# GogoRit/llm-inference-lab

Measured on AMD Instinct MI355X. Metric: accepted tokens/sec + acceptance-rate, Llama-3.2-3B/1B K=4 @1/2/4/8 GPU, higher is better.
Workload: dtype bf16; 1 GPU; llama-3.2-3b target + llama-3.2-1b draft, K=4, batch 1/GPU, greedy, prompt 32 ids, hipGraph step, weights: synthetic; K=4, batch_per_gpu=1, global_batch=1, prompt_len=32, parallelism=dp1

## Files before the change

llm-inference-lab_amd/csrc/debug_env.h:

```cpp
#pragma once

namespace sd {
namespace debug_env {

constexpr const char* kNoPersist = "SPECDEC_NO_PERSIST";
constexpr const char* kPersistMaxT = "SPECDEC_PERSIST_MAX_T";
constexpr const char* kPersistTaps = "SPECDEC_PERSIST_TAPS";
constexpr const char* kPersistDropWg = "SPECDEC_PERSIST_TEST_DROP_WG";
constexpr const char* kNoFwd0Select = "SPECDEC_NO_FWD0_SELECT";
constexpr const char* kMaxPassTokens = "SPECDEC_MAX_PASS_TOKENS";
constexpr const char* kNoDirect = "SPECDEC_NO_DIRECT";
constexpr const char* kNoPipe = "SPECDEC_NO_PIPE";
constexpr const char* kNoAttnSplit = "SPECDEC_NO_ATTN_SPLIT";
constexpr const char* kNoGemmPrefill = "SPECDEC_NO_GEMM_PREFILL";
constexpr const char* kPrefillMinTokens = "SPECDEC_PREFILL_MIN_TOKENS";
constexpr const char* kMedusaPerHead = "SPECDEC_MEDUSA_PER_HEAD";
constexpr const char* kGemvTimeline = "SPECDEC_GEMV_TIMELINE";
constexpr const char* kProbeHot = "SPECDEC_PROBE_HOT";
constexpr const char* kProbeNoXstat = "SPECDEC_PROBE_NO_XSTAT";

}
}
```

llm-inference-lab_amd/csrc/engine.hip:

```cpp

#include <hip/hip_runtime.h>

#include <stdlib.h>

#include <new>
#include <vector>

#include "engine.h"
#include "persist.h"
#include "prefill_gemm.h"

struct sd_model {
  sd_model_config cfg;
  std::vector<sd_layer_weights> layers;
  uint16_t* k_cache = nullptr;
  uint16_t* v_cache = nullptr;
  int B = 0, Lmax = 0;
  const int32_t* block_table = nullptr;
  int page_shift = 0, max_pages = 0, n_pages = 0;
  uint16_t* x = nullptr;
  uint16_t* q = nullptr;
  uint16_t* attn = nullptr;
  uint16_t* act = nullptr;
  int32_t* probe_pos = nullptr;
  float* attn_ws = nullptr;
  unsigned* attn_cnt = nullptr;
  float* xstat = nullptr;
  float* part_val = nullptr;
  int small_t = sd::kGemvMaxT;
  int max_t = sd::kGemvMaxT;
  int* part_idx = nullptr;
  int head_grid = 0;
  const int32_t* skip_k = nullptr;
  int skip_i = 0;
  std::vector<const void*> packed;
  std::vector<const float*> scales;
  const void* mat(int index, const void* row_major) const { return packed.empty() ? row_major : packed[index]; }
  int is_packed() const { return packed.empty() ? 0 : 1; }
  int w8() const { return scales.empty() ? 0 : 1; }
  const float* scale(int index) const { return scales.empty() ? nullptr : scales[index]; }
  int persist_t = 0;
  bool persist_taps = true;
  sd::PersistOp* p_ops = nullptr;
  unsigned long long* p_gran = nullptr;
  unsigned p_gran_parity = 0;
  unsigned* p_sync = nullptr;
  unsigned long long* p_debug = nullptr;
  void* prefill_ws = nullptr;
  int prefill_backend = SD_PREFILL_AUTO;
  int64_t prefill_count[4] = {0, 0, 0, 0};
  sd::NativePlan native_plan;
  void* score_ws = nullptr;
  unsigned* host_status = nullptr;
  int persist_cap = 0;
  int len_hint = 0;
  int ctx_limit = 0;
  ~sd_model() {
// ... 53 lines not shown
  const int d = c.d_model, HqD = c.n_heads * c.head_dim, ff = c.d_ff;
  const struct { const uint16_t* x; int x_stride; uint16_t* out; int out_stride; } rows[5] = {
      {m->x, d, m->q, HqD}, {m->attn, HqD, m->x, d}, {m->x, d, m->act, ff}, {m->act, ff, m->x, d}, {m->x, d, nullptr, 0}};
  a.x = rows[which].x;
  a.x_stride = rows[which].x_stride;
  a.out = rows[which].out;
  a.out_stride = rows[which].out_stride;
  a.out_dtype = SD_BF16;
  if (which == 4) {
    a.part_val = m->part_val;
    a.part_idx = m->part_idx;
  }
  return a;
}

static int forward_pass(sd_model* m, const int32_t* tokens, int tok_stride, const int32_t* pos_base,
                        int pos_off, int row0, int b0, int Bc, int Mc, int32_t* ids_out, int ids_stride,
                        void* logits_out, int logits_dtype, int logits_stride, int skip_head,
                        hipStream_t st) {
  const sd_model_config& c = m->cfg;
  const int T = Bc * Mc;
  const int d = c.d_model, Hq = c.n_heads, Hkv = c.n_kv_heads, D = c.head_dim, ff = c.d_ff;
  const bool llama = (c.arch == SD_ARCH_LLAMA);

  if (persist_pass_ok(m, T, Bc, Mc)) {
    PersistArgs pa{};
    pa.ops = m->p_ops;
    pa.n_ops = 4 * c.n_layers + (skip_head ? 0 : 1);
    pa.d_model = d; pa.n_q_heads = Hq; pa.n_kv_heads = Hkv; pa.head_dim = D; pa.d_ff = ff; pa.vocab = c.vocab;
    pa.n_layers = c.n_layers; pa.max_pos = c.max_pos;
    pa.norm_eps = c.norm_eps;
    pa.attn_scale = 1.0f / sqrtf(static_cast<float>(D));
    pa.tok_emb = c.tok_emb;
    pa.rope_cos = c.rope_cos;
    pa.rope_sin = c.rope_sin;
    pa.tokens = tokens + static_cast<size_t>(b0) * tok_stride;
    pa.tok_stride = tok_stride;
    pa.pos_base = pos_base + b0;
    pa.pos_off = pos_off;
    pa.B = Bc;
    pa.M = Mc;
    const size_t row_off = static_cast<size_t>(row0 + b0) * Hkv * m->Lmax * D;
    pa.k_cache = m->k_cache + row_off;
    pa.v_cache = m->v_cache + row_off;
    pa.layer_kv = static_cast<size_t>(m->B) * Hkv * m->Lmax * D;
    pa.l_max = m->Lmax;
    pa.logits = logits_out;
    pa.logits_dtype = logits_dtype;
    pa.logits_stride = logits_stride;
    pa.part_val = m->part_val;
    pa.part_idx = m->part_idx;
    pa.x = m->x; pa.q = m->q; pa.attn = m->attn; pa.act = m->act;
    pa.gran = m->p_gran;
    pa.gran_parity = m->p_gran_parity;
    pa.sync = m->p_sync;
    pa.host_status = m->host_status;
    pa.skip_k = m->skip_k;
    pa.skip_i = m->skip_i;
    pa.taps = (m->persist_taps || skip_head) ? 1 : 0;
    pa.debug_ts = m->p_debug;
    if (int rc = launch_persist_forward(pa, st)) return rc;
    if (skip_head) return 0;
    m->head_grid = kPersistCUs;
    if (ids_out) {
      if (int rc = launch_argmax_finalize(m->part_val, m->part_idx, T, m->head_grid, Mc, ids_stride,
                                          ids_out + static_cast<size_t>(b0) * ids_stride, st, m->skip_k, m->skip_i))
        return rc;
    }
    return 0;
  }

  EmbedArgs e{};
  e.tok_emb = c.tok_emb;
  e.pos_emb = llama ? nullptr : c.pos_emb;
  e.tokens = tokens + static_cast<size_t>(b0) * tok_stride;
  e.tok_stride = tok_stride;
  e.pos_base = pos_base + b0;
  e.pos_off = pos_off;
  e.M = Mc;
  e.T = T;
  e.d = d;
  e.vocab = c.vocab;
  e.max_pos = c.max_pos;
  e.x = m->x;
  e.skip_k = m->skip_k;
  e.skip_i = m->skip_i;
  if (int rc = launch_embed(e, st)) return rc;

  const bool paged = m->block_table != nullptr;
  const size_t layer_kv = paged ? (static_cast<size_t>(m->n_pages) * Hkv * D << m->page_shift) : static_cast<size_t>(m->B) * Hkv * m->Lmax * D;
  const size_t row_kv = paged ? 0 : static_cast<size_t>(row0 + b0) * Hkv * m->Lmax * D;
  const int32_t* bt = paged ? m->block_table + static_cast<size_t>(row0 + b0) * m->max_pages : nullptr;
  const float* stat_in = nullptr;
  int stat_n = 0;
  auto publish = [&](GemvArgs& prod) {
    stat_in = nullptr;
    if (m->xstat && gemm_resid_publishes_stats(prod)) {
      prod.xstat_out = m->xstat;
      stat_in = m->xstat;
      int ppw = 1;
      stat_n = gemv_grid(prod, &ppw);
    }
  };
  for (int l = 0; l < c.n_layers; ++l) {
    uint16_t* kc = m->k_cache + l * layer_kv + row_kv;
    uint16_t* vc = m->v_cache + l * layer_kv + row_kv;
    auto layer_args = [&](int which) {
      GemvArgs g = matrix_args(m, 4 * l + which);
      g.T = T;
// ... 837 lines not shown
    if (int rc = launch_argmax_finalize(m->part_val, m->part_idx, B * K, grid, K, K + 1, s->st.verify_tok + 1, st_t)) return rc;
    if (int rc = launch_medusa_commit(s->st, st_t)) return rc;
  } else if (!s->draft && s->heads.empty()) {
    if (int rc = model_forward(s->target, s->st.verify_tok, K + 1, s->st.cur_len, 0, 0, B, 1, s->st.draft_ids, 2, nullptr, SD_BF16, 0, st_t))
      return rc;
    if (int rc = launch_medusa_fill(s->st, st_t)) return rc;
  }
  if (two) {
    SD_HIP_CHECK(hipEventRecord(s->ev_fork, st_t));
    SD_HIP_CHECK(hipStreamWaitEvent(st_d, s->ev_fork, 0));
  }
  struct TapsGuard {
    sd_model* m; bool saved;
    TapsGuard(sd_model* m_, bool v) : m(m_), saved(m_ ? m_->persist_taps : false) { if (m) m->persist_taps = v; }
    ~TapsGuard() { if (m) m->persist_taps = saved; }
  } taps_guard(s->draft, s->draft_taps);
  const bool fwd0_select = s->draft && s->st.fwd0_w && B == 1 && persist_pass_ok(s->draft, 2, 1, 2);
  const bool one_pass_d = s->draft && B * 2 <= s->draft->max_t;
  const auto finalize = [&](int M, int i, int32_t* ids, const int32_t* skip_k, int skip_i) -> int {
    if (one_pass_d)
      return launch_draft_finalize(s->draft->part_val, s->draft->part_idx, s->draft->head_grid, M, i, ids, s->st, skip_k, skip_i, st_d);
    return 0;
  };
  const bool spec = s->spec != 0;
  const int V = s->target->cfg.vocab;
  uint16_t* const q_pass = spec ? static_cast<uint16_t*>(s->spec_p) : nullptr;
  int32_t* const ids_d = (one_pass_d || spec) ? nullptr : s->st.draft_ids;
  for (int i = 0; s->draft && i < K; ++i) {
    const int M = (i == 0) ? 2 : 1;
    const int32_t* toks = (i == 0) ? s->st.tok2 : s->st.next_tok;
    const int off = (i == 0) ? -1 : i;
    s->draft->skip_k = (s->st.adaptive && i >= 1) ? s->st.k_active : nullptr;
    s->draft->skip_i = i;
    int rc_f;
    if (i == 0 && fwd0_select) {
      s->draft->skip_k = s->st.fwd0_w;
      s->draft->skip_i = 1;
      rc_f = model_forward(s->draft, toks, 2, s->st.cur_len, -1, 0, B, 2, ids_d, 2, q_pass, SD_BF16, 0, st_d);
      if (!rc_f && !spec) rc_f = finalize(2, 0, s->st.draft_ids, s->st.fwd0_w, 1);
      if (!rc_f) {
        s->draft->skip_k = s->st.fwd0_w + 1;
        rc_f = model_forward(s->draft, toks + 1, 2, s->st.cur_len, 0, 0, B, 1, ids_d ? ids_d + 1 : nullptr, 2, spec ? q_pass + V : nullptr,
                             SD_BF16, 0, st_d);
      }
      if (!rc_f && !spec) rc_f = finalize(1, 0, s->st.draft_ids + 1, s->st.fwd0_w + 1, 1);
    } else {
      rc_f = model_forward(s->draft, toks, M, s->st.cur_len, off, 0, B, M, ids_d, 2, q_pass, SD_BF16, 0, st_d);
      if (!rc_f && !spec) rc_f = finalize(M, i, s->st.draft_ids, s->draft->skip_k, i);
    }
    s->draft->skip_k = nullptr;
    if (rc_f) return rc_f;
    if (spec && s->spec_top_k > 0) {
      if (int rc = launch_spec_draft_draw_shaped(s->st, q_pass, M, M - 1, s->spec_q, i, V, s->temperature, s->spec_top_k, s->spec_top_p,
                                                 s->seed, s->draw, s->stream_id, st_d))
        return rc;
    } else if (spec) {
      if (int rc = launch_spec_draft_draw(s->st, q_pass, M, M - 1, s->spec_q, i, V, s->temperature, s->seed, s->draw, s->stream_id, st_d)) return rc;
    } else if (!one_pass_d) {
      if (int rc = launch_draft_next(M, i, s->st, st_d)) return rc;
    }
  }
  if (two) {
    SD_HIP_CHECK(hipEventRecord(s->ev_join, st_d));
    SD_HIP_CHECK(hipStreamWaitEvent(st_t, s->ev_join, 0));
  }
  const unsigned* const st_word_d = (s->draft && s->draft->p_sync) ? s->draft->p_sync + 1 : nullptr;
  const unsigned* const st_word_t = s->target->p_sync ? s->target->p_sync + 1 : nullptr;
  const bool tail = !s->sample && !spec && verify_tail_fits(s->st) && B * (K + 1) <= s->target->max_t;
  if (int rc = model_forward(s->target, s->st.verify_tok, K + 1, s->st.cur_len, 0, 0, B, K + 1, tail ? nullptr : s->st.target_ids,
                             K + 1, s->sample ? s->logits : (spec ? s->spec_p : nullptr), SD_BF16, 0, st_t))
    return rc;
  if (tail) {
    if (int rc = launch_verify_tail(s->st, s->target->part_val, s->target->part_idx, s->target->head_grid, s->mode, s->host_record, s->rec,
                                    s->step_counter, st_word_d, st_word_t, st_t))
      return rc;
    if (!s->heads.empty())
      if (int rc = enqueue_medusa_heads(s, st_t)) return rc;
    return 0;
  }
  if (s->sample) {
    if (int rc = launch_accept_len(s->st, st_t)) return rc;
    if (int rc = launch_sample_step(s->st, s->logits, s->target->cfg.vocab, s->temperature, s->top_k, s->top_p, s->seed,
                                    s->draw, s->stream_id, st_t))
      return rc;
  }
  if (spec && s->spec_top_k > 0) {
    if (int rc = launch_spec_step_shaped(s->st, s->spec_p, s->spec_q, V, s->temperature, s->spec_top_k, s->spec_top_p, s->seed, s->draw,
                                         s->stream_id, s->spec_flags, s->spec_flags + static_cast<size_t>(B) * (K + 1), st_t))
      return rc;
  } else if (spec) {
    if (int rc = launch_spec_step(s->st, s->spec_p, s->spec_q, V, s->temperature, s->seed, s->draw, s->stream_id, s->spec_flags,
                                  s->spec_flags + static_cast<size_t>(B) * (K + 1), st_t))
      return rc;
  }
// ... 394 lines not shown
}

extern "C" long sd_specdec_launches(const sd_specdec* s) { return s ? s->launches : 0; }

extern "C" int sd_specdec_wait(sd_specdec* s, long launch_index) {
  clear_error();
  SD_REQUIRE(s, "specdec_wait: NULL");
  SD_REQUIRE(launch_index >= 0 && launch_index < s->launches && launch_index + 2 >= s->launches,
             "specdec_wait: step %ld is not one of the last two launches (%ld launched)", launch_index, s->launches);
  SD_HIP_CHECK(hipEventSynchronize(s->ev_done[launch_index & 1]));
  return 0;
}

extern "C" int sd_specdec_sync(sd_specdec* s, void* stream) {
  clear_error();
  (void)s;
  SD_HIP_CHECK(hipStreamSynchronize(static_cast<hipStream_t>(stream)));
  return 0;
}

extern "C" const int32_t* sd_specdec_record(const sd_specdec* s) { return s ? s->host_record : nullptr; }

extern "C" int sd_specdec_record_ints(const sd_specdec* s) { return s ? s->rec : 0; }
```

llm-inference-lab_amd/csrc/kernels.h:

```cpp
#pragma once

#include <vector>

#include "common.h"
#include "debug_env.h"

namespace sd {

enum GemvPrologue { PRO_NONE = 0, PRO_RMSNORM = 1, PRO_LAYERNORM = 2 };
enum GemvEpilogue { EPI_QKV_ROPE = 0, EPI_RESID = 1, EPI_SWIGLU = 2, EPI_GELU = 3, EPI_ARGMAX = 4 };

constexpr int kGemvMaxT = 9;
constexpr int kSkinnyMaxT = 128;
static_assert(kSkinnyMaxT <= 255, "GemvArgs::T / M are 8-bit fields");

struct GemvArgs {
  const void* W;
  const void* x;
  void* out;
  const void* norm_w;
  const void* norm_b;
  const void* bias;
  const int32_t* x_row;
  const int32_t* skip_k;
// ... 90 lines not shown

struct AttnArgs {
  const void* q;
  const void* k_cache;
  const void* v_cache;
  void* out;
  const int32_t* pos_base;
  const int32_t* skip_k;
  int pos_off;
  int l_max;
  float scale;
  unsigned M : 8, n_q_heads : 8, n_kv_heads : 8, n_split : 8;
  unsigned head_dim : 8, page_shift : 8, skip_i : 4;
  int B;
  float* split_ws;
  unsigned* split_cnt;
  int split_slots;
  const int32_t* block_table;
};
int launch_attention(const AttnArgs& a, hipStream_t st);
constexpr int kAttnSplitSlots = 1024;
size_t attention_split_ws_bytes(int head_dim);

struct EmbedArgs {
  const void* tok_emb;
  const void* pos_emb;
  const int32_t* tokens;
  int tok_stride;
  const int32_t* pos_base;
  int pos_off, M, T, d, vocab, max_pos;
  void* x;
  const int32_t* skip_k;
  int skip_i;
};
int launch_embed(const EmbedArgs& a, hipStream_t st);

int launch_argmax_finalize(const float* part_val, const int* part_idx, int T, int grid, int M,
                           int ids_stride, int32_t* ids_out, hipStream_t st, const int32_t* skip_k = nullptr, int skip_i = 0);

}
```

llm-inference-lab_amd/csrc/misc.hip:

```cpp

#include "kernels.h"
#include "engine.h"

namespace sd {

__global__ __launch_bounds__(256) void embed_kernel(const EmbedArgs a) {
  SD_SKIP_IF_INACTIVE(a.skip_k, a.skip_i);
  const int t = blockIdx.x;
  const int b = t / a.M, m = t - b * a.M;
  int tok = a.tokens[b * a.tok_stride + m];
  tok = tok < 0 ? 0 : (tok >= a.vocab ? a.vocab - 1 : tok);
  const uint4* src = reinterpret_cast<const uint4*>(static_cast<const uint16_t*>(a.tok_emb) + static_cast<size_t>(tok) * a.d);
  uint4* dst = reinterpret_cast<uint4*>(static_cast<uint16_t*>(a.x) + static_cast<size_t>(t) * a.d);
  const int nvec = a.d >> 3;
  if (!a.pos_emb) {
    for (int v = threadIdx.x; v < nvec; v += blockDim.x) dst[v] = src[v];
    return;
  }
  int pos = a.pos_base[b] + a.pos_off + m;
  pos = pos < 0 ? 0 : (pos >= a.max_pos ? a.max_pos - 1 : pos);
  const uint4* ps = reinterpret_cast<const uint4*>(static_cast<const uint16_t*>(a.pos_emb) + static_cast<size_t>(pos) * a.d);
  for (int v = threadIdx.x; v < nvec; v += blockDim.x) {
    const uint4 e = src[v], p = ps[v];
    const uint32_t ew[4] = {e.x, e.y, e.z, e.w}, pw[4] = {p.x, p.y, p.z, p.w};
    uint32_t o[4];
#pragma unroll
    for (int j = 0; j < 4; ++j) {
      const float lo = __uint_as_float(ew[j] << 16) + __uint_as_float(pw[j] << 16);
      const float hi = __uint_as_float(ew[j] & 0xffff0000u) + __uint_as_float(pw[j] & 0xffff0000u);
      o[j] = static_cast<uint32_t>(float_to_bf16_bits(lo)) | (static_cast<uint32_t>(float_to_bf16_bits(hi)) << 16);
    }
    dst[v] = make_uint4(o[0], o[1], o[2], o[3]);
  }
}

int launch_embed(const EmbedArgs& a, hipStream_t st) {
  SD_REQUIRE(a.d % 8 == 0, "embed: d=%d must be a multiple of 8", a.d);
  hipLaunchKernelGGL(embed_kernel, dim3(a.T), dim3(256), 0, st, a);
  SD_LAUNCH_CHECK();
  return 0;
}

__device__ __forceinline__ int fold_partials(const float* pv, const int* pi, int grid, int lane) {
  float v = -INFINITY;
  int i = 0x7fffffff;
  for (int s = lane; s < grid; s += kWave) {
    const float sv = pv[s];
    const int si = pi[s];
    if (argmax_better(sv, si, v, i)) { v = sv; i = si; }
  }
  wave_reduce_argmax(v, i);
  return i;
}

__global__ __launch_bounds__(kWave) void argmax_finalize_kernel(const float* part_val, const int* part_idx,
                                                                int grid, int M, int ids_stride,
                                                                int32_t* ids, const int32_t* skip_k, int skip_i) {
  SD_SKIP_IF_INACTIVE(skip_k, skip_i);
  const int t = blockIdx.x, lane = threadIdx.x;
  const int i = fold_partials(part_val + static_cast<size_t>(t) * grid, part_idx + static_cast<size_t>(t) * grid, grid, lane);
  if (lane == 0) {
    if (M > 0) {
      const int b = t / M, m = t - b * M;
      ids[b * ids_stride + m] = i;
    } else {
      const int j = t / -M, b = t + j * M;
      ids[b * ids_stride + j] = i;
    }
  }
}

int launch_argmax_finalize(const float* part_val, const int* part_idx, int T, int grid, int M,
                           int ids_stride, int32_t* ids_out, hipStream_t st, const int32_t* skip_k, int skip_i) {
  hipLaunchKernelGGL(argmax_finalize_kernel, dim3(T), dim3(kWave), 0, st, part_val, part_idx, grid, M,
                     ids_stride, ids_out, skip_k, skip_i);
// ... 348 lines not shown
```

llm-inference-lab_amd/csrc/persist.h:

```cpp
#pragma once

#include "kernels.h"

namespace sd {

enum PersistKind { POP_QKV = 0, POP_OUT = 1, POP_GATEUP = 2, POP_DOWN = 3, POP_HEAD = 4 };

struct PersistOp {
  const void* W;
  const void* norm_w;
  unsigned pair_bytes;
  int n_pairs, ppw, tile_pairs;
  int K;
  int kind, layer;
  int pad_[5];
};
static_assert(sizeof(PersistOp) == 64, "PersistOp is read as whole 64-byte records");

constexpr int kPersistMaxT = 8;
constexpr int kPersistCUs = 256;
constexpr int kPersistMaxQkvTiles = 4;

enum PersistEdge { PE_X = 0, PE_QKV = 1, PE_ATTN = 2, PE_X2 = 3, PE_ACT = 4 };

// ... 10 lines not shown
  const int32_t* pos_base;
  int pos_off;
  int B, M;
  void* k_cache;
  void* v_cache;
  size_t layer_kv;
  int l_max;
  void* logits;
  int logits_dtype, logits_stride;
  float* part_val;
  int* part_idx;
  void* x;
  void* q;
  void* attn;
  void* act;
  unsigned long long* gran;
  unsigned gran_parity;
  unsigned off_edge[5];
  unsigned gran_unit;
  unsigned* sync;
  unsigned* host_status;
  const int32_t* skip_k;
  int skip_i;
  unsigned lds_rope, lds_resid, lds_part, lds_attn, lds_u, lds_ring;
  unsigned ring_bytes;
  unsigned u_stride;
  unsigned resid_ppw;
  int taps;
  unsigned long long* debug_ts;
};

size_t persist_workspace_bytes(const sd_model_config& c);
constexpr unsigned kGranUnitMax = 528;
bool persist_model_ok(const sd_model_config& c, bool packed, bool w8, int n_cus);
inline bool persist_cache_ok(int l_max) { return l_max >= 8 && l_max % 8 == 0; }
int persist_max_tokens(const sd_model_config& c);
int launch_persist_forward(PersistArgs a, hipStream_t st);

}
```

llm-inference-lab_amd/csrc/persist.hip:

```cpp

#include <stdlib.h>

#include "gemv_device.h"
#include "persist.h"

#ifndef SD_P_DIAG
#define SD_P_DIAG 0
#endif

namespace sd {
namespace {

constexpr unsigned kPiece = 1024;
constexpr int kChunk = 16;
constexpr int kBackoff = 2;
constexpr int kSplitSweep = 2048;
constexpr int kLeadInUnits = 96;
constexpr unsigned kUniformSites = 13;
constexpr unsigned kTimeoutTicks = 50u * 1000u * 100u;
constexpr int kPartT = kPersistMaxT;

enum : unsigned { ST_LOADER = 1u, ST_LANDED = 2u, ST_USEQ = 4u, ST_PART = 8u, ST_GRANULE = 16u, ST_ATTN = 32u };

struct PCtl {
  unsigned landed;
  unsigned consumed[3];
  unsigned abort_;
  unsigned u_seq;
  unsigned done[3];
  unsigned lead_done;
  unsigned a_seq;
  unsigned a_done[3];
  unsigned a_merged;
  unsigned g2_seq;
  unsigned a2_seq;
  unsigned nsum[2];
  unsigned nseq[2];
  unsigned gathering;
};

typedef const PersistOp __attribute__((address_space(4)))* cops_t;

__device__ __forceinline__ unsigned lds_ld(const unsigned* p) {
  const unsigned v = __hip_atomic_load(p, __ATOMIC_RELAXED, __HIP_MEMORY_SCOPE_WORKGROUP);
  asm volatile("" ::: "memory");
  return static_cast<unsigned>(__builtin_amdgcn_readfirstlane(static_cast<int>(v)));
}
__device__ __forceinline__ void lds_st(unsigned* p, unsigned v) {
  asm volatile("" ::: "memory");
  __hip_atomic_store(p, v, __ATOMIC_RELAXED, __HIP_MEMORY_SCOPE_WORKGROUP);
}

__device__ __forceinline__ void dma_piece(const char* sbase, unsigned voff, unsigned lds_dst) {
  asm volatile("s_mov_b32 m0, %2\n\ts_nop 0\n\tglobal_load_lds_dwordx4 %0, %1 nt" ::"v"(voff), "s"(sbase), "s"(lds_dst) : "memory");
}

template <bool STAMPS, bool TAPS>
struct PCtxT {
  static constexpr bool kStamps = STAMPS;
  static constexpr bool kTaps = TAPS;
  const PersistArgs* a;
  unsigned char* smem;
// ... 490 lines not shown
    for (int k = 0; k < NC; ++k)
#pragma unroll
      for (int j = 0; j < LPC; ++j) x[k][j] = __hip_atomic_load(p[k][j], __ATOMIC_RELAXED, __HIP_MEMORY_SCOPE_AGENT);
  };
  auto complete = [&](const unsigned long long (&x)[NC][LPC]) {
    bool ok = true;
#pragma unroll
    for (int k = 0; k < NC; ++k)
#pragma unroll
      for (int j = 0; j < LPC; ++j) {
        v[k][j] = static_cast<unsigned>(x[k][j]);
        ok &= static_cast<unsigned>(x[k][j] >> 32) == tag;
      }
    return __all(ok) != 0;
  };
  for (unsigned spins = 1;; ++spins) {
    issue(xa);
    if (complete(xa)) return true;
    __builtin_amdgcn_s_sleep(kBackoff);
    if ((spins & 255u) == 0u && expired<3>(c)) { give_up(c, ST_GRANULE); return false; }
  }
}

template <int HC, class C>
__device__ __forceinline__ bool gather_norm_rows(const C& c, const OpView& o, int edge, bool from_embedding, const ConsState& st, int ts, int t0, int tstep,
                                                 int me) {
  const PersistArgs& a = *c.a;
  const int npt = a.d_model >> 1;
  const unsigned* nw = static_cast<const unsigned*>(o.norm_w);
  unsigned wv[HC][16];
#pragma unroll
  for (int hc = 0; hc < HC; ++hc)
#pragma unroll
    for (int j = 0; j < 16; ++j) {
      const int idx = hc * 1024 + j * 64 + c.lane;
      wv[hc][j] = nw[idx < npt ? idx : npt - 1];
    }
  for (int t = t0; t < c.T; t += tstep) {
    unsigned v[HC][16];
    if (from_embedding) {
      const int b = t / a.M, m = t - b * a.M;
      int tok = a.tokens[b * a.tok_stride + m];
      tok = tok < 0 ? 0 : (tok >= a.vocab ? a.vocab - 1 : tok);
      const unsigned* row = reinterpret_cast<const unsigned*>(static_cast<const uint16_t*>(a.tok_emb) + static_cast<size_t>(tok) * a.d_model);
#pragma unroll
      for (int hc = 0; hc < HC; ++hc)
#pragma unroll
        for (int j = 0; j < 16; ++j) {
          const int idx = hc * 1024 + j * 64 + c.lane;
          v[hc][j] = row[idx < npt ? idx : npt - 1];
        }
#pragma unroll
      for (int hc = 0; hc < HC; ++hc)
#pragma unroll
        for (int j = 0; j < 16; ++j)
          if (hc * 1024 + j * 64 + c.lane >= npt) v[hc][j] = 0u;
    } else {
      if (!sweep<HC>(c, edge_base(a, o.layer, edge), static_cast<unsigned>(t) * npt, npt, edge_tag(c, o.layer, edge), v)) return false;
#pragma unroll
      for (int hc = 0; hc < HC; ++hc)
#pragma unroll
        for (int j = 0; j < 16; ++j)
          if (hc * 1024 + j * 64 + c.lane >= npt) v[hc][j] = 0u;
    }
    f32x2_t s2 = {0.f, 0.f};
// ... 13 lines not shown
#pragma unroll
      for (int j = 0; j < 16; ++j) {
        const int idx = hc * 1024 + j * 64 + c.lane;
        if (idx < npt) dst[idx] = rmsnorm_pair(v[hc][j], rs, wv[hc][j]);
      }
  }
  return true;
}

template <int HC, class C>
__device__ __forceinline__ bool gather_norm_half(const C& c, const OpView& o, int edge, bool from_embedding, const ConsState& st, int ts, int me, unsigned seq) {
  const PersistArgs& a = *c.a;
  constexpr int LP = HC == 1 ? 8 : 16;
  const int npt = a.d_model >> 1, half = npt >> 1, c0 = (me == 2) ? half : 0;
  const unsigned* nw = static_cast<const unsigned*>(o.norm_w) + c0;
  unsigned wv[LP];
#pragma unroll
  for (int j = 0; j < LP; ++j) {
    const int idx = j * 64 + c.lane;
    wv[j] = nw[idx < half ? idx : half - 1];
  }
  unsigned v[1][LP];
  if (from_embedding) {
    int tok = a.tokens[0];
    tok = tok < 0 ? 0 : (tok >= a.vocab ? a.vocab - 1 : tok);
    const unsigned* row = reinterpret_cast<const unsigned*>(static_cast<const uint16_t*>(a.tok_emb) + static_cast<size_t>(tok) * a.d_model) + c0;
#pragma unroll
    for (int j = 0; j < LP; ++j) {
      const int idx = j * 64 + c.lane;
      v[0][j] = row[idx < half ? idx : half - 1];
    }
  } else {
    if (!sweep<1, LP>(c, edge_base(a, o.layer, edge), static_cast<unsigned>(c0), half, edge_tag(c, o.layer, edge), v)) return false;
  }
  f32x2_t s2 = {0.f, 0.f};
#pragma unroll
  for (int j = 0; j < LP; ++j) {
    if (j * 64 + c.lane >= half) v[0][j] = 0u;
    const f32x2_t f = bf16x2_unpack(v[0][j]);
    s2 += f * f;
  }
  const float mine = wave_reduce_sum(s2.x + s2.y);
  lds_st(&c.ctl->nsum[me - 1], __float_as_uint(mine));
  lds_st(&c.ctl->nseq[me - 1], seq);
  if (!wait_word<1>(c, &c.ctl->nseq[2 - me], seq, ST_USEQ)) return false;
  const float other = __uint_as_float(lds_ld(&c.ctl->nsum[2 - me]));
  const float sq = (me == 1) ? mine + other : other + mine;
// ... 309 lines not shown
  const int n_units = a.B * a.n_q_heads;
  const int unit = unit_of_cu(c.cu, n_units);

  if (cw == 0) {
    const OpView o0 = load_op(c, 0);
    const int half = a.head_dim >> 1;
    float2* rope = reinterpret_cast<float2*>(c.smem + a.lds_rope);
    for (int tile = 0; tile < o0.n_tiles; ++tile) {
      const int p = o0.p_lo + tile * o0.tile_pairs + L.jp;
      float2 cs = {1.f, 0.f};
      if (L.tok_ok && L.jp < o0.tile_pairs && p < o0.n_pairs && L.pos >= 0 && L.pos < a.max_pos) {
        const int i = p % half;
        cs.x = a.rope_cos[static_cast<size_t>(L.pos) * half + i];
        cs.y = a.rope_sin[static_cast<size_t>(L.pos) * half + i];
      }
      rope[tile * 64 + lane] = cs;
    }
    unsigned* res = reinterpret_cast<unsigned*>(c.smem + a.lds_resid);
    const int npt = a.d_model >> 1;
    for (int it = lane; it < c.T * static_cast<int>(a.resid_ppw); it += 64) {
      const int t = it / a.resid_ppw, j = it - t * a.resid_ppw;
      const int p = c.cu * a.resid_ppw + j;
      const int b = t / a.M, m = t - b * a.M;
      int tok = a.tokens[b * a.tok_stride + m];
      tok = tok < 0 ? 0 : (tok >= a.vocab ? a.vocab - 1 : tok);
      res[it] = (p < npt) ? reinterpret_cast<const unsigned*>(static_cast<const uint16_t*>(a.tok_emb) + static_cast<size_t>(tok) * a.d_model)[p] : 0u;
    }
  }

  for (int i = 0; i < a.n_ops; ++i) {
    const OpView o = load_op(c, i);
    const bool normed = o.kind == POP_QKV || o.kind == POP_GATEUP || o.kind == POP_HEAD;
    if (cw == 1) stamp(c, 12 * i + 0);
    if (cw == 1) lds_st(&c.ctl->gathering, 1u);
    bool ok = true;
    const bool rows_shared = c.T > 1;
    if (normed) {
      const bool halves = !rows_shared && (a.d_model & 255) == 0;
      if (cw == 1 || (cw == 2 && (rows_shared || halves))) {
        const int edge = (o.kind == POP_GATEUP) ? PE_X2 : PE_X;
        const bool emb = (o.kind == POP_QKV && o.layer == 0) || (o.kind == POP_HEAD && a.n_layers == 0);
        if (halves) ok = gather_norm_half<HC>(c, o, edge, emb, st, cw == 1 ? 12 * i : -1, cw, static_cast<unsigned>(i + 1));
        else ok = gather_norm_rows<HC>(c, o, edge, emb, st, cw == 1 ? 12 * i : -1, cw - 1, rows_shared ? 2 : 1, cw);
        if (ok && (rows_shared || halves)) {
          if (cw == 2) lds_st(&c.ctl->g2_seq, static_cast<unsigned>(i + 1));
          else ok = wait_word<1>(c, &c.ctl->g2_seq, static_cast<unsigned>(i + 1), ST_USEQ);
        }
// ... 39 lines not shown
    }
    if (cw == 0) stamp(c, 12 * i + 2);
    if (o.kind == POP_QKV && unit >= 0) {
      if (!attention_unit<D>(c, cw, o.layer, unit / a.n_q_heads, unit % a.n_q_heads, st, 12 * i)) return;
      if (cw == 0) stamp(c, 12 * i + 3);
    }
  }
  if (cw == 0 && a.n_ops > 0 && c.ops[a.n_ops - 1].kind == POP_HEAD) {
    float bv = st.best_v;
    int bi = st.best_i;
#pragma unroll
    for (int off = 4; off > 0; off >>= 1) {
      const float ov = __shfl_xor(bv, off, 64);
      const int oi = __shfl_xor(bi, off, 64);
      if (argmax_better(ov, oi, bv, bi)) { bv = ov; bi = oi; }
    }
    if (L.tok_ok && L.jp == 0) {
      a.part_val[static_cast<size_t>(L.t) * kPersistCUs + c.cu] = bv;
      a.part_idx[static_cast<size_t>(L.t) * kPersistCUs + c.cu] = bi;
    }
  }
}

template <int D, int HC, bool STAMPS, bool SEL, bool TAPS>
__global__ __launch_bounds__(256) void persist_forward_kernel(const PersistArgs a) {
  extern __shared__ __attribute__((aligned(16))) unsigned char smem[];
  SD_SKIP_IF_INACTIVE(a.skip_k, a.skip_i);
  const int tid = threadIdx.x;
  const int wave = __builtin_amdgcn_readfirstlane(tid >> 6);
  if (tid < 64) reinterpret_cast<unsigned*>(smem)[tid] = 0u;
  for (int i = tid; i < 4 * D; i += 256) reinterpret_cast<unsigned*>(smem + a.lds_attn + 2 * a.M * D * 2)[i] = 0u;
  const unsigned launch = __hip_atomic_load(a.sync, __ATOMIC_RELAXED, __HIP_MEMORY_SCOPE_AGENT);
  __syncthreads();
  PCtxT<STAMPS, TAPS> c;
  c.a = &a;
  c.smem = smem;
  c.ctl = reinterpret_cast<PCtl*>(smem);
  c.t_start = __builtin_amdgcn_s_memrealtime();
  c.lane = tid & 63;
  c.cu = blockIdx.x;
  c.T = a.B * a.M;
  c.tag0 = launch << 9;
  c.ops = (cops_t)a.ops;
  unsigned long long clk0 = 0;
  if (STAMPS && a.debug_ts && wave == 1) clk0 = __builtin_amdgcn_s_memtime();
  if (wave == 0) loader_role(c);
  else consumer_role<D, HC>(c, wave - 1);
  if (STAMPS && a.debug_ts && wave == 1 && c.lane == 0) {
    unsigned long long* d = a.debug_ts + static_cast<size_t>(c.cu) * (12 * a.n_ops + 4) + 12 * a.n_ops;
    d[0] = c.t_start;
    d[1] = clk0;
    d[2] = __builtin_amdgcn_s_memrealtime();
    d[3] = __builtin_amdgcn_s_memtime();
// ... 75 lines not shown
  n += (2 * persist_gran_parity(c) * 8 + 255) & ~static_cast<size_t>(255);
  return n;
}

template <int D, int HC, bool STAMPS, bool SEL, bool TAPS>
static int launch_inst(const PersistArgs& a, size_t smem, hipStream_t st) {
  static unsigned long long attr_set = 0;
  if (int rc = opt_in_dynamic_lds(reinterpret_cast<const void*>(&persist_forward_kernel<D, HC, STAMPS, SEL, TAPS>), static_cast<int>(kLdsBytes), attr_set)) return rc;
  const int grid = getenv(debug_env::kPersistDropWg) ? kPersistCUs - 1 : kPersistCUs;
  hipLaunchKernelGGL((persist_forward_kernel<D, HC, STAMPS, SEL, TAPS>), dim3(grid), dim3(256), smem, st, a);
  SD_LAUNCH_CHECK();
  return 0;
}
template <int D, int HC>
static int launch_one(const PersistArgs& a, size_t smem, hipStream_t st) {
  if (a.debug_ts) return launch_inst<D, HC, true, false, true>(a, smem, st);
  if (a.taps) return a.skip_k ? launch_inst<D, HC, false, true, true>(a, smem, st) : launch_inst<D, HC, false, false, true>(a, smem, st);
  return a.skip_k ? launch_inst<D, HC, false, true, false>(a, smem, st) : launch_inst<D, HC, false, false, false>(a, smem, st);
}

int launch_persist_forward(PersistArgs a, hipStream_t st) {
  const int T = a.B * a.M;
  SD_REQUIRE(T >= 1 && T <= kPersistMaxT && a.M <= 8, "persist: T=%d M=%d out of range", T, a.M);
  SD_REQUIRE(a.B * a.n_q_heads <= kPersistCUs, "persist: %d attention units exceed the CUs", a.B * a.n_q_heads);
  SD_REQUIRE(a.l_max >= 8 && a.l_max % 8 == 0, "persist: cache rows of %d positions (need a multiple of 8)", a.l_max);
  const int HqD = a.n_q_heads * a.head_dim;
  const LdsPlan p = plan_lds(a.d_model, HqD, a.d_ff, a.head_dim, T, a.M);
  SD_REQUIRE(p.ok, "persist: T=%d rows do not fit the LDS next to a 64 KiB ring", T);
  a.lds_rope = p.rope;
  a.lds_resid = p.resid;
  a.lds_part = p.part;
  a.lds_attn = p.attn;
  a.lds_u = p.u;
  a.lds_ring = p.ring;
  a.ring_bytes = p.ring_bytes;
  a.u_stride = p.u_stride;
  a.resid_ppw = gemv_geometry(a.d_model / 2, HqD).ppw;
  a.gran_unit = kGranUnitMax;
  size_t off = 0;
  a.off_edge[PE_X] = static_cast<unsigned>(off); off += edge_storage(a.d_model / 2, a.gran_unit);
  a.off_edge[PE_QKV] = static_cast<unsigned>(off); off += edge_storage((a.n_q_heads + 2 * a.n_kv_heads) * a.head_dim / 2, a.gran_unit);
  a.off_edge[PE_ATTN] = static_cast<unsigned>(off); off += edge_storage(HqD / 2, a.gran_unit);
  a.off_edge[PE_X2] = static_cast<unsigned>(off); off += edge_storage(a.d_model / 2, a.gran_unit);
  a.off_edge[PE_ACT] = static_cast<unsigned>(off); off += edge_storage(a.d_ff / 2, a.gran_unit);
  SD_REQUIRE(off <= a.gran_parity, "persist: granule buffer too small");
  const size_t smem = kLdsBytes;
// ... 7 lines not shown
```

Baseline: 699.0 tokens/s.

## Fold draft argmax finalize into the next forward's embedding entry

Stops launching a separate argmax-finalize kernel after each draft forward. The reduction of head partials is deferred into the next forward, either the next draft step or the target verify pass. There it runs inside the embed kernel or at entry to the persistent kernel, which writes the draft token buffers and uses the token directly for embedding. This removes a kernel launch and graph node per draft step, at the cost of a small serial reduction at kernel entry and more complex gating logic. The new path is on by default and can be turned off with an environment variable.

```diff
diff --git a/llm-inference-lab_amd/csrc/debug_env.h b/llm-inference-lab_amd/csrc/debug_env.h
--- a/llm-inference-lab_amd/csrc/debug_env.h
+++ b/llm-inference-lab_amd/csrc/debug_env.h
@@ -8,6 +8,7 @@
 constexpr const char* kPersistTaps = "SPECDEC_PERSIST_TAPS";
 constexpr const char* kPersistDropWg = "SPECDEC_PERSIST_TEST_DROP_WG";
 constexpr const char* kNoFwd0Select = "SPECDEC_NO_FWD0_SELECT";
+constexpr const char* kNoFoldFinalize = "SPECDEC_NO_FOLD_FINALIZE";
 constexpr const char* kMaxPassTokens = "SPECDEC_MAX_PASS_TOKENS";
 constexpr const char* kNoDirect = "SPECDEC_NO_DIRECT";
 constexpr const char* kNoPipe = "SPECDEC_NO_PIPE";
diff --git a/llm-inference-lab_amd/csrc/engine.hip b/llm-inference-lab_amd/csrc/engine.hip
--- a/llm-inference-lab_amd/csrc/engine.hip
+++ b/llm-inference-lab_amd/csrc/engine.hip
@@ -33,6 +33,7 @@
   int head_grid = 0;
   const int32_t* skip_k = nullptr;
   int skip_i = 0;
+  sd::FoldSrc fold{};
   std::vector<const void*> packed;
   std::vector<const float*> scales;
   const void* mat(int index, const void* row_major) const { return packed.empty() ? row_major : packed[index]; }
@@ -132,6 +133,7 @@
   const int T = Bc * Mc;
   const int d = c.d_model, Hq = c.n_heads, Hkv = c.n_kv_heads, D = c.head_dim, ff = c.d_ff;
   const bool llama = (c.arch == SD_ARCH_LLAMA);
+  SD_REQUIRE(!m->fold.part_val || (b0 == 0 && Bc * Mc <= m->max_t), "forward: a fold source needs the forward to be one pass");
 
   if (persist_pass_ok(m, T, Bc, Mc)) {
     PersistArgs pa{};
@@ -167,6 +169,7 @@
     pa.host_status = m->host_status;
     pa.skip_k = m->skip_k;
     pa.skip_i = m->skip_i;
+    pa.fold = m->fold;
     pa.taps = (m->persist_taps || skip_head) ? 1 : 0;
     pa.debug_ts = m->p_debug;
     if (int rc = launch_persist_forward(pa, st)) return rc;
@@ -195,6 +198,7 @@
   e.x = m->x;
   e.skip_k = m->skip_k;
   e.skip_i = m->skip_i;
+  e.fold = m->fold;
   if (int rc = launch_embed(e, st)) return rc;
 
   const bool paged = m->block_table != nullptr;
@@ -1078,6 +1082,30 @@
       return launch_draft_finalize(s->draft->part_val, s->draft->part_idx, s->draft->head_grid, M, i, ids, s->st, skip_k, skip_i, st_d);
     return 0;
   };
+  const bool fold_d = one_pass_d && !s->spec && !s->sample && !getenv(debug_env::kNoFoldFinalize);
+  const bool fold_v = fold_d && B * (K + 1) <= s->target->max_t;
+  FoldSrc pend{};
+  const auto defer_finalize = [&](int M, int i, const int32_t* gate, const int32_t* gate_alt, int gate_i) {
+    pend.part_val = s->draft->part_val;
+    pend.part_idx = s->draft->part_idx;
+    pend.grid = s->draft->head_grid;
+    pend.M = M;
+    pend.i = i;
+    pend.tok_m = (i + 1 < K) ? 0 : K;
+    pend.gate_i = gate_i;
+    pend.gate = gate;
+    pend.gate_alt = gate_alt;
+    pend.draft_ids = s->st.draft_ids;
+    pend.draft_tok = s->st.draft_tok;
+    pend.verify_tok = s->st.verify_tok;
+    pend.next_tok = s->st.next_tok;
+    pend.K = K;
+  };
+  struct FoldGuard {
+    sd_model* m;
+    FoldGuard(sd_model* m_, FoldSrc& f) : m(m_) { m->fold = f; f = FoldSrc{}; }
+    ~FoldGuard() { m->fold = FoldSrc{}; }
+  };
   const bool spec = s->spec != 0;
   const int V = s->target->cfg.vocab;
   uint16_t* const q_pass = spec ? static_cast<uint16_t*>(s->spec_p) : nullptr;
@@ -1086,6 +1114,8 @@
     const int M = (i == 0) ? 2 : 1;
     const int32_t* toks = (i == 0) ? s->st.tok2 : s->st.next_tok;
     const int off = (i == 0) ? -1 : i;
+    const bool fold_i = fold_d && (i + 1 < K || fold_v);
+    FoldGuard fold_guard(s->draft, pend);
     s->draft->skip_k = (s->st.adaptive && i >= 1) ? s->st.k_active : nullptr;
     s->draft->skip_i = i;
     int rc_f;
@@ -1093,16 +1123,18 @@
       s->draft->skip_k = s->st.fwd0_w;
       s->draft->skip_i = 1;
       rc_f = model_forward(s->draft, toks, 2, s->st.cur_len, -1, 0, B, 2, ids_d, 2, q_pass, SD_BF16, 0, st_d);
-      if (!rc_f && !spec) rc_f = finalize(2, 0, s->st.draft_ids, s->st.fwd0_w, 1);
+      if (!rc_f && !spec && !fold_i) rc_f = finalize(2, 0, s->st.draft_ids, s->st.fwd0_w, 1);
       if (!rc_f) {
         s->draft->skip_k = s->st.fwd0_w + 1;
         rc_f = model_forward(s->draft, toks + 1, 2, s->st.cur_len, 0, 0, B, 1, ids_d ? ids_d + 1 : nullptr, 2, spec ? q_pass + V : nullptr,
                              SD_BF16, 0, st_d);
       }
-      if (!rc_f && !spec) rc_f = finalize(1, 0, s->st.draft_ids + 1, s->st.fwd0_w + 1, 1);
+      if (!rc_f && !spec && !fold_i) rc_f = finalize(1, 0, s->st.draft_ids + 1, s->st.fwd0_w + 1, 1);
+      if (!rc_f && fold_i) defer_finalize(2, 0, s->st.fwd0_w, s->st.fwd0_w + 1, 1);
     } else {
       rc_f = model_forward(s->draft, toks, M, s->st.cur_len, off, 0, B, M, ids_d, 2, q_pass, SD_BF16, 0, st_d);
-      if (!rc_f && !spec) rc_f = finalize(M, i, s->st.draft_ids, s->draft->skip_k, i);
+      if (!rc_f && !spec && !fold_i) rc_f = finalize(M, i, s->st.draft_ids, s->draft->skip_k, i);
+      if (!rc_f && fold_i) defer_finalize(M, i, s->draft->skip_k, nullptr, i);
     }
     s->draft->skip_k = nullptr;
     if (rc_f) return rc_f;
@@ -1123,9 +1155,12 @@
   const unsigned* const st_word_d = (s->draft && s->draft->p_sync) ? s->draft->p_sync + 1 : nullptr;
   const unsigned* const st_word_t = s->target->p_sync ? s->target->p_sync + 1 : nullptr;
   const bool tail = !s->sample && !spec && verify_tail_fits(s->st) && B * (K + 1) <= s->target->max_t;
-  if (int rc = model_forward(s->target, s->st.verify_tok, K + 1, s->st.cur_len, 0, 0, B, K + 1, tail ? nullptr : s->st.target_ids,
-                             K + 1, s->sample ? s->logits : (spec ? s->spec_p : nullptr), SD_BF16, 0, st_t))
-    return rc;
+  {
+    FoldGuard fold_guard(s->target, pend);
+    if (int rc = model_forward(s->target, s->st.verify_tok, K + 1, s->st.cur_len, 0, 0, B, K + 1, tail ? nullptr : s->st.target_ids,
+                               K + 1, s->sample ? s->logits : (spec ? s->spec_p : nullptr), SD_BF16, 0, st_t))
+      return rc;
+  }
   if (tail) {
     if (int rc = launch_verify_tail(s->st, s->target->part_val, s->target->part_idx, s->target->head_grid, s->mode, s->host_record, s->rec,
                                     s->step_counter, st_word_d, st_word_t, st_t))
@@ -1566,3 +1601,39 @@
 extern "C" const int32_t* sd_specdec_record(const sd_specdec* s) { return s ? s->host_record : nullptr; }
 
 extern "C" int sd_specdec_record_ints(const sd_specdec* s) { return s ? s->rec : 0; }
+
+extern "C" int sd_specdec_debug_words(sd_specdec* s, int poison, int32_t* out) {
+  clear_error();
+  SD_REQUIRE(s, "specdec_debug_words: NULL");
+  SD_HIP_CHECK(hipDeviceSynchronize());
+  const int B = s->B, K = s->K;
+  if (poison) {
+    std::vector<int32_t> w(static_cast<size_t>(B) * (K + 1), poison);
+    SD_HIP_CHECK(hipMemcpy(s->st.draft_tok, w.data(), sizeof(int32_t) * B * K, hipMemcpyHostToDevice));
+    SD_HIP_CHECK(hipMemcpy(s->st.next_tok, w.data(), sizeof(int32_t) * B, hipMemcpyHostToDevice));
+    SD_HIP_CHECK(hipMemcpy(s->st.draft_ids, w.data(), sizeof(int32_t) * B * 2, hipMemcpyHostToDevice));
+    for (int b = 0; b < B; ++b)
+      SD_HIP_CHECK(hipMemcpy(s->st.verify_tok + static_cast<size_t>(b) * (K + 1) + 1, w.data(), sizeof(int32_t) * K, hipMemcpyHostToDevice));
+    const size_t n_part = static_cast<size_t>(sd::kSkinnyMaxT) * sd::kMaxPartials;
+    std::vector<float> pv(n_part, INFINITY);
+    std::vector<int32_t> pi(n_part, poison);
+    for (sd_model* m : {s->draft, s->target}) {
+      if (!m || !m->part_val) continue;
+      SD_HIP_CHECK(hipMemcpy(m->part_val, pv.data(), n_part * sizeof(float), hipMemcpyHostToDevice));
+      SD_HIP_CHECK(hipMemcpy(m->part_idx, pi.data(), n_part * sizeof(int32_t), hipMemcpyHostToDevice));
+    }
+  }
+  if (out) {
+    SD_HIP_CHECK(hipMemcpy(out, s->st.draft_tok, sizeof(int32_t) * B * K, hipMemcpyDeviceToHost));
+    SD_HIP_CHECK(hipMemcpy(out + B * K, s->st.verify_tok, sizeof(int32_t) * B * (K + 1), hipMemcpyDeviceToHost));
+    SD_HIP_CHECK(hipMemcpy(out + B * (2 * K + 1), s->st.next_tok, sizeof(int32_t) * B, hipMemcpyDeviceToHost));
+  }
+  return 0;
+}
+
+extern "C" int sd_specdec_debug_graph_nodes(const sd_specdec* s) {
+  if (!s || !s->graph) return 0;
+  size_t n = 0;
+  if (hipGraphGetNodes(s->graph, nullptr, &n) != hipSuccess) return -1;
+  return static_cast<int>(n);
+}
diff --git a/llm-inference-lab_amd/csrc/fold_device.h b/llm-inference-lab_amd/csrc/fold_device.h
--- /dev/null
+++ b/llm-inference-lab_amd/csrc/fold_device.h
@@ -0,0 +1,76 @@
+#pragma once
+
+#include "kernels.h"
+
+namespace sd {
+
+#if defined(__HIPCC__)
+
+__device__ __forceinline__ int fold_partials(const float* pv, const int* pi, int grid, int lane) {
+  float v = -INFINITY;
+  int i = 0x7fffffff;
+  for (int s = lane; s < grid; s += kWave) {
+    const float sv = pv[s];
+    const int si = pi[s];
+    if (argmax_better(sv, si, v, i)) { v = sv; i = si; }
+  }
+  wave_reduce_argmax(v, i);
+  return i;
+}
+
+struct FoldForm {
+  int m_prev;
+  int id_slot;
+};
+__device__ __forceinline__ FoldForm fold_src_form(const FoldSrc& f) {
+  const int g = f.gate ? *f.gate : 0x7fffffff;
+  const int g_alt = f.gate_alt ? *f.gate_alt : -0x7fffffff;
+  if (g_alt > f.gate_i) return FoldForm{1, 1};
+  return FoldForm{g > f.gate_i ? f.M : 0, f.M - 1};
+}
+
+__device__ __forceinline__ int fold_src_token(const FoldSrc& f, int b, int lane, FoldForm& form) {
+  const size_t t_a = static_cast<size_t>(b) * f.M + f.M - 1, t_b = static_cast<size_t>(b);
+  const float* pv_a = f.part_val + t_a * f.grid;
+  const int* pi_a = f.part_idx + t_a * f.grid;
+  if (!f.gate_alt) {
+    const int d = fold_partials(pv_a, pi_a, f.grid, lane);
+    form = fold_src_form(f);
+    return d;
+  }
+  const float* pv_b = f.part_val + t_b * f.grid;
+  const int* pi_b = f.part_idx + t_b * f.grid;
+  float va = -INFINITY, vb = -INFINITY;
+  int ia = 0x7fffffff, ib = 0x7fffffff;
+  for (int s = lane; s < f.grid; s += kWave) {
+    const float sa = pv_a[s], sb = pv_b[s];
+    const int ja = pi_a[s], jb = pi_b[s];
+    if (argmax_better(sa, ja, va, ia)) { va = sa; ia = ja; }
+    if (argmax_better(sb, jb, vb, ib)) { vb = sb; ib = jb; }
+  }
+  form = fold_src_form(f);
+  float v = form.id_slot == 1 && form.m_prev == 1 ? vb : va;
+  int i = form.id_slot == 1 && form.m_prev == 1 ? ib : ia;
+  wave_reduce_argmax(v, i);
+  return i;
+}
+
+__device__ __forceinline__ void fold_src_store(const FoldSrc& f, int b, const FoldForm& form, int d) {
+  if (form.m_prev == 0) return;
+  f.draft_ids[b * 2 + form.id_slot] = d;
+  f.draft_tok[b * f.K + f.i] = d;
+  f.verify_tok[b * (f.K + 1) + f.i + 1] = d;
+  f.next_tok[b] = d;
+}
+
+__device__ __forceinline__ void fold_src_first_token(const FoldSrc& f, int b, int lane) {
+  if (f.M != 2) return;
+  const size_t t = static_cast<size_t>(b) * 2;
+  const int d = fold_partials(f.part_val + t * f.grid, f.part_idx + t * f.grid, f.grid, lane);
+  const FoldForm form = fold_src_form(f);
+  if (lane == 0 && form.m_prev == 2) f.draft_ids[b * 2] = d;
+}
+
+#endif
+
+}
diff --git a/llm-inference-lab_amd/csrc/kernels.h b/llm-inference-lab_amd/csrc/kernels.h
--- a/llm-inference-lab_amd/csrc/kernels.h
+++ b/llm-inference-lab_amd/csrc/kernels.h
@@ -136,6 +136,23 @@
 constexpr int kAttnSplitSlots = 1024;
 size_t attention_split_ws_bytes(int head_dim);
 
+struct FoldSrc {
+  const float* part_val;
+  const int* part_idx;
+  int grid;
+  int M;
+  int i;
+  int tok_m;
+  int gate_i;
+  const int32_t* gate;
+  const int32_t* gate_alt;
+  int32_t* draft_ids;
+  int32_t* draft_tok;
+  int32_t* verify_tok;
+  int32_t* next_tok;
+  int K;
+};
+
 struct EmbedArgs {
   const void* tok_emb;
   const void* pos_emb;
@@ -146,6 +163,7 @@
   void* x;
   const int32_t* skip_k;
   int skip_i;
+  FoldSrc fold;
 };
 int launch_embed(const EmbedArgs& a, hipStream_t st);
 
diff --git a/llm-inference-lab_amd/csrc/misc.hip b/llm-inference-lab_amd/csrc/misc.hip
--- a/llm-inference-lab_amd/csrc/misc.hip
+++ b/llm-inference-lab_amd/csrc/misc.hip
@@ -1,14 +1,34 @@
 
 #include "kernels.h"
 #include "engine.h"
+#include "fold_device.h"
 
 namespace sd {
 
 __global__ __launch_bounds__(256) void embed_kernel(const EmbedArgs a) {
-  SD_SKIP_IF_INACTIVE(a.skip_k, a.skip_i);
   const int t = blockIdx.x;
   const int b = t / a.M, m = t - b * a.M;
-  int tok = a.tokens[b * a.tok_stride + m];
+  __shared__ int s_tok;
+  int tok;
+  if (a.fold.part_val && m == a.fold.tok_m) {
+    const int wave = threadIdx.x / kWave, lane = threadIdx.x % kWave;
+    if (wave == 0) {
+      FoldForm form;
+      const int d = fold_src_token(a.fold, b, lane, form);
+      if (lane == 0) {
+        fold_src_store(a.fold, b, form, d);
+        s_tok = form.m_prev ? d : a.tokens[b * a.tok_stride + m];
+      }
+    } else if (wave == 1) {
+      fold_src_first_token(a.fold, b, lane);
+    }
+    SD_SKIP_IF_INACTIVE(a.skip_k, a.skip_i);
+    __syncthreads();
+    tok = s_tok;
+  } else {
+    SD_SKIP_IF_INACTIVE(a.skip_k, a.skip_i);
+    tok = a.tokens[b * a.tok_stride + m];
+  }
   tok = tok < 0 ? 0 : (tok >= a.vocab ? a.vocab - 1 : tok);
   const uint4* src = reinterpret_cast<const uint4*>(static_cast<const uint16_t*>(a.tok_emb) + static_cast<size_t>(tok) * a.d);
   uint4* dst = reinterpret_cast<uint4*>(static_cast<uint16_t*>(a.x) + static_cast<size_t>(t) * a.d);
@@ -39,18 +59,6 @@
   hipLaunchKernelGGL(embed_kernel, dim3(a.T), dim3(256), 0, st, a);
   SD_LAUNCH_CHECK();
   return 0;
-}
-
-__device__ __forceinline__ int fold_partials(const float* pv, const int* pi, int grid, int lane) {
-  float v = -INFINITY;
-  int i = 0x7fffffff;
-  for (int s = lane; s < grid; s += kWave) {
-    const float sv = pv[s];
-    const int si = pi[s];
-    if (argmax_better(sv, si, v, i)) { v = sv; i = si; }
-  }
-  wave_reduce_argmax(v, i);
-  return i;
 }
 
 __global__ __launch_bounds__(kWave) void argmax_finalize_kernel(const float* part_val, const int* part_idx,
diff --git a/llm-inference-lab_amd/csrc/persist.h b/llm-inference-lab_amd/csrc/persist.h
--- a/llm-inference-lab_amd/csrc/persist.h
+++ b/llm-inference-lab_amd/csrc/persist.h
@@ -56,6 +56,7 @@
   unsigned* host_status;
   const int32_t* skip_k;
   int skip_i;
+  FoldSrc fold;
   unsigned lds_rope, lds_resid, lds_part, lds_attn, lds_u, lds_ring;
   unsigned ring_bytes;
   unsigned u_stride;
diff --git a/llm-inference-lab_amd/csrc/persist.hip b/llm-inference-lab_amd/csrc/persist.hip
--- a/llm-inference-lab_amd/csrc/persist.hip
+++ b/llm-inference-lab_amd/csrc/persist.hip
@@ -3,6 +3,7 @@
 
 #include "gemv_device.h"
 #include "persist.h"
+#include "fold_device.h"
 
 #ifndef SD_P_DIAG
 #define SD_P_DIAG 0
@@ -37,7 +38,9 @@
   unsigned nsum[2];
   unsigned nseq[2];
   unsigned gathering;
+  unsigned fold_tok[kPersistMaxT];
 };
+static_assert(sizeof(PCtl) <= 256, "the kernel clears the first 256 bytes of LDS as the control words");
 
 typedef const PersistOp __attribute__((address_space(4)))* cops_t;
 
@@ -574,6 +577,13 @@
   }
 }
 
+template <class C>
+__device__ __forceinline__ int pass_token(const C& c, int b, int m) {
+  const PersistArgs& a = *c.a;
+  if (a.fold.part_val) return static_cast<int>(lds_ld(&c.ctl->fold_tok[b]));
+  return a.tokens[b * a.tok_stride + m];
+}
+
 template <int HC, class C>
 __device__ __forceinline__ bool gather_norm_rows(const C& c, const OpView& o, int edge, bool from_embedding, const ConsState& st, int ts, int t0, int tstep,
                                                  int me) {
@@ -592,7 +602,7 @@
     unsigned v[HC][16];
     if (from_embedding) {
       const int b = t / a.M, m = t - b * a.M;
-      int tok = a.tokens[b * a.tok_stride + m];
+      int tok = pass_token(c, b, m);
       tok = tok < 0 ? 0 : (tok >= a.vocab ? a.vocab - 1 : tok);
       const unsigned* row = reinterpret_cast<const unsigned*>(static_cast<const uint16_t*>(a.tok_emb) + static_cast<size_t>(tok) * a.d_model);
 #pragma unroll
@@ -652,7 +662,7 @@
   }
   unsigned v[1][LP];
   if (from_embedding) {
-    int tok = a.tokens[0];
+    int tok = pass_token(c, 0, 0);
     tok = tok < 0 ? 0 : (tok >= a.vocab ? a.vocab - 1 : tok);
     const unsigned* row = reinterpret_cast<const unsigned*>(static_cast<const uint16_t*>(a.tok_emb) + static_cast<size_t>(tok) * a.d_model) + c0;
 #pragma unroll
@@ -1008,7 +1018,7 @@
       const int t = it / a.resid_ppw, j = it - t * a.resid_ppw;
       const int p = c.cu * a.resid_ppw + j;
       const int b = t / a.M, m = t - b * a.M;
-      int tok = a.tokens[b * a.tok_stride + m];
+      int tok = pass_token(c, b, m);
       tok = tok < 0 ? 0 : (tok >= a.vocab ? a.vocab - 1 : tok);
       res[it] = (p < npt) ? reinterpret_cast<const unsigned*>(static_cast<const uint16_t*>(a.tok_emb) + static_cast<size_t>(tok) * a.d_model)[p] : 0u;
     }
@@ -1094,13 +1104,32 @@
   }
 }
 
+__device__ __forceinline__ void fold_at_entry(const PersistArgs& a, PCtl* ctl, int wave, int lane) {
+  if (wave == 0) {
+    for (int b = 0; b < a.B; ++b) {
+      FoldForm form;
+      const int d = fold_src_token(a.fold, b, lane, form);
+      if (lane == 0) {
+        if (blockIdx.x == 0) fold_src_store(a.fold, b, form, d);
+        ctl->fold_tok[b] = static_cast<unsigned>(form.m_prev ? d : a.tokens[b * a.tok_stride]);
+      }
+    }
+  } else if (wave == 1 && blockIdx.x == 0) {
+    for (int b = 0; b < a.B; ++b) fold_src_first_token(a.fold, b, lane);
+  }
+}
+
 template <int D, int HC, bool STAMPS, bool SEL, bool TAPS>
 __global__ __launch_bounds__(256) void persist_forward_kernel(const PersistArgs a) {
   extern __shared__ __attribute__((aligned(16))) unsigned char smem[];
-  SD_SKIP_IF_INACTIVE(a.skip_k, a.skip_i);
+  if (!a.fold.part_val || blockIdx.x != 0) SD_SKIP_IF_INACTIVE(a.skip_k, a.skip_i);
   const int tid = threadIdx.x;
   const int wave = __builtin_amdgcn_readfirstlane(tid >> 6);
   if (tid < 64) reinterpret_cast<unsigned*>(smem)[tid] = 0u;
+  if (a.fold.part_val) {
+    fold_at_entry(a, reinterpret_cast<PCtl*>(smem), wave, tid & 63);
+    if (blockIdx.x == 0) SD_SKIP_IF_INACTIVE(a.skip_k, a.skip_i);
+  }
   for (int i = tid; i < 4 * D; i += 256) reinterpret_cast<unsigned*>(smem + a.lds_attn + 2 * a.M * D * 2)[i] = 0u;
   const unsigned launch = __hip_atomic_load(a.sync, __ATOMIC_RELAXED, __HIP_MEMORY_SCOPE_AGENT);
   __syncthreads();
@@ -1222,6 +1251,7 @@
 int launch_persist_forward(PersistArgs a, hipStream_t st) {
   const int T = a.B * a.M;
   SD_REQUIRE(T >= 1 && T <= kPersistMaxT && a.M <= 8, "persist: T=%d M=%d out of range", T, a.M);
+  SD_REQUIRE(!a.fold.part_val || (a.M == 1 && a.fold.tok_m == 0), "persist: a fold source needs a 1-token pass (M=%d)", a.M);
   SD_REQUIRE(a.B * a.n_q_heads <= kPersistCUs, "persist: %d attention units exceed the CUs", a.B * a.n_q_heads);
   SD_REQUIRE(a.l_max >= 8 && a.l_max % 8 == 0, "persist: cache rows of %d positions (need a multiple of 8)", a.l_max);
   const int HqD = a.n_q_heads * a.head_dim;
```

After: 698.2 tokens/s. No clear change (-0.1%).
